# MOj0/vpt

Hardware: AMD Instinct MI355X
Metric: volume samples/s, MCM 512^3 @ 1920x1080 (higher is better)
Workload: dtype f32

## Files before the change

### vpt_amd/csrc/vpt_device.h

```cpp
#pragma once
#include <hip/hip_runtime.h>
#include <stdint.h>
#include "vpt_variants.h"

#define VPT_DEV __device__ __forceinline__

struct f3 { float x, y, z; };
struct f2 { float x, y; };

VPT_DEV float vmin(float a, float b) { return fminf(a, b); }
VPT_DEV float vmax(float a, float b) { return fmaxf(a, b); }
VPT_DEV float vclamp01(float x) { return vmin(vmax(x, 0.0f), 1.0f); }
VPT_DEV float mixf(float a, float b, float t) { return fmaf(b, t, a * (1.0f - t)); }
VPT_DEV f3 mix3(f3 a, f3 b, float t) { return f3{ mixf(a.x, b.x, t), mixf(a.y, b.y, t), mixf(a.z, b.z, t) }; }
VPT_DEV float dot3(f3 a, f3 b) { return fmaf(a.z, b.z, fmaf(a.y, b.y, a.x * b.x)); }
VPT_DEV float length3(f3 a) { return sqrtf(dot3(a, a)); }
VPT_DEV f3 sub3(f3 a, f3 b) { return f3{ a.x - b.x, a.y - b.y, a.z - b.z }; }
VPT_DEV f3 madd3(f3 p, float t, f3 d) { return f3{ fmaf(t, d.x, p.x), fmaf(t, d.y, p.y), fmaf(t, d.z, p.z) }; }
VPT_DEV float lerpf(float a, float b, float f) { return fmaf(f, b - a, a); }
VPT_DEV float4 lerp4(float4 a, float4 b, float f) {
    return make_float4(lerpf(a.x, b.x, f), lerpf(a.y, b.y, f), lerpf(a.z, b.z, f), lerpf(a.w, b.w, f));
}

VPT_DEV float rcp_nr(float x) {
// ... 347 lines not shown
        const uint32_t s0 = (uint32_t)(uintptr_t)a & 2u, s1 = ((uint32_t)(uintptr_t)a + 50u) & 2u;
        return norm16_blend<SNORM>(plane16_aligned(a - s0, s0), plane16_aligned(a + 50 - s1, s1), fx, fy, fz);
    }
    return norm16_blend<SNORM>(plane16(a), plane16(a + 50), fx, fy, fz);
}
template <bool WIDE>
VPT_DEV const uint8_t *record_addr(const DevVolume &v, const LdsTables &t, uint32_t x, uint32_t y, uint32_t z) {
    if (WIDE) return v.records + ((uint64_t)(t.tx[x] + t.ty[y]) * v.rec_col_bytes + (z << 2));
    return v.records + (uint32_t)(t.tx[x] + t.ty[y] + (z << 2));
}
VPT_DEV float record_blend(uint32_t lo, uint32_t hi, float fx, float fy, float fz) {
    float c000 = cvt_ubyte<0>(lo), c100 = cvt_ubyte<1>(lo), c010 = cvt_ubyte<2>(lo), c110 = cvt_ubyte<3>(lo);
    float c001 = cvt_ubyte<0>(hi), c101 = cvt_ubyte<1>(hi), c011 = cvt_ubyte<2>(hi), c111 = cvt_ubyte<3>(hi);
    float c00 = lerpf(c000, c100, fx), c10 = lerpf(c010, c110, fx);
    float c01 = lerpf(c001, c101, fx), c11 = lerpf(c011, c111, fx);
    float c0 = lerpf(c00, c10, fy), c1 = lerpf(c01, c11, fy);
    return lerpf(c0, c1, fz) * VPT_INV255;
}
VPT_DEV uint64_t record_load(const uint8_t *a) {
    uint64_t w;
    __builtin_memcpy(&w, __builtin_assume_aligned(a, 4), 8);
    return w;
}
VPT_DEV uint32_t boundary_cell(const DevVolume &v, f3 p, float &out_fa, float &out_fb) {
    const float fnx = v.fnx, fny = v.fny, fnz = v.fnz, hx = v.hx, hy = v.hy, hz = v.hz;
    const uint32_t face = v.atlas_face, sh = v.atlas_shift;
    const bool ox = (p.x > 1.0f) || (p.x < 0.0f);
    const bool oy = (p.y > 1.0f) || (p.y < 0.0f);
    const unsigned long long act = __builtin_amdgcn_ballot_w64(true);
    const unsigned long long bx = __builtin_amdgcn_ballot_w64(p.x > 1.0f) | __builtin_amdgcn_ballot_w64(p.x < 0.0f);
    const unsigned long long by = __builtin_amdgcn_ballot_w64(p.y > 1.0f) | __builtin_amdgcn_ballot_w64(p.y < 0.0f);
    uint32_t a, b, idx; float fa, fb;
    if (bx == act) {
        linear_cell(p.y, fny, hy, a, fa); linear_cell(p.z, fnz, hz, b, fb);
        idx = (p.x > 1.0f ? face : 0u) + ((b << sh) + a);
    } else if (bx == 0ull && by == act) {
        linear_cell(p.x, fnx, hx, a, fa); linear_cell(p.z, fnz, hz, b, fb);
        idx = (p.y > 1.0f ? 3u * face : 2u * face) + ((b << sh) + a);
    } else if (bx == 0ull && by == 0ull) {
        linear_cell(p.x, fnx, hx, a, fa); linear_cell(p.y, fny, hy, b, fb);
        idx = (p.z > 1.0f ? 5u * face : 4u * face) + ((b << sh) + a);
    } else {
        const bool oxy = ox || oy;
        const float pa = ox ? p.y : p.x, pb = oxy ? p.z : p.y;
        linear_cell(pa, ox ? fny : fnx, ox ? hy : hx, a, fa);
        linear_cell(pb, oxy ? fnz : fny, oxy ? hz : hy, b, fb);
        const float pk = ox ? p.x : (oy ? p.y : p.z);
        const uint32_t f = (ox ? 0u : (oy ? 2u : 4u)) + (pk > 1.0f ? 1u : 0u);
        idx = f * face + ((b << sh) + a);
    }
    out_fa = fa; out_fb = fb;
    return idx;
}
template <bool NEAREST>
VPT_DEV uint32_t boundary_cell_lane(const DevVolume &v, f3 p, float &out_fa, float &out_fb) {
    const float fnx = v.fnx, fny = v.fny, fnz = v.fnz, hx = v.hx, hy = v.hy, hz = v.hz;
    const bool ox = (p.x > 1.0f) || (p.x < 0.0f);
    const bool oy = (p.y > 1.0f) || (p.y < 0.0f);
    const bool oxy = ox || oy;
    const float pa = ox ? p.y : p.x, pb = oxy ? p.z : p.y;
    const float fna = ox ? fny : fnx, ha = ox ? hy : hx, fnb = oxy ? fnz : fny, hb = oxy ? hz : hy;
    uint32_t a, b; float fa = 0.0f, fb = 0.0f;
    if (NEAREST) { a = nearest_cell(pa, fna, ha); b = nearest_cell(pb, fnb, hb); }
    else { linear_cell(pa, fna, ha, a, fa); linear_cell(pb, fnb, hb, b, fb); }
    const float pk = ox ? p.x : (oy ? p.y : p.z);
    const uint32_t f = (ox ? 0u : (oy ? 2u : 4u)) + (pk > 1.0f ? 1u : 0u);
    out_fa = fa; out_fb = fb;
    return f * v.atlas_face + ((b << v.atlas_shift) + a);
}
template <bool SNORM = false>
VPT_DEV float boundary_blend(uint32_t w, float fa, float fb) {
    float c00 = byte_tap<SNORM, 0>(w), c10 = byte_tap<SNORM, 1>(w), c01 = byte_tap<SNORM, 2>(w), c11 = byte_tap<SNORM, 3>(w);
    const float r = lerpf(lerpf(c00, c10, fa), lerpf(c01, c11, fa), fb);
    return SNORM ? r : r * VPT_INV255;
}
template <int V>
VPT_DEV f2 sample_boundary_rg(const DevVolume &v, f3 p) {
    constexpr bool NEAREST = (V & VPT_V_NEAREST) != 0, RG = (V & VPT_V_RG) != 0, F32 = (V & (VPT_V_F32 | VPT_V_NORM16)) != 0, SNORM = (V & VPT_V_SNORM) != 0;
    float fa, fb;
    const uint32_t idx = boundary_cell_lane<NEAREST>(v, p, fa, fb);
    fa = cell_weight<V>(fa); fb = cell_weight<V>(fb);
    float val[2] = { 0.0f, 0.0f };
#pragma unroll
    for (int c = 0; c < (RG ? 2 : 1); c++) {
        const uint32_t cell = idx + (uint32_t)c * 6u * v.atlas_face;
        if (F32) {
            const float4 t = ((const float4 *)v.atlas)[cell];
            val[c] = NEAREST ? t.x : lerpf(lerpf(t.x, t.y, fa), lerpf(t.z, t.w, fa), fb);
        } else {
            const uint32_t w = v.atlas[cell];
            if (SNORM) val[c] = NEAREST ? snorm_byte<0>(w) : boundary_blend<true>(w, fa, fb);
            else val[c] = NEAREST ? cvt_ubyte<0>(w) * VPT_INV255 : boundary_blend(w, fa, fb);
        }
    }
    return f2{ val[0], val[1] };
}
VPT_DEV float sample_volume_boundary(const DevVolume &v, f3 p) {
    float fa, fb;
    const uint32_t idx = boundary_cell(v, p, fa, fb);
    return boundary_blend(v.atlas[idx], fa, fb);
}
template <int V>
VPT_DEV f2 sample_volume_rg(const DevVolume &v, const LdsTables &t, f3 p) {
    constexpr bool WIDE = (V & VPT_V_WIDE) != 0;
    constexpr bool RG = (V & VPT_V_RG) != 0;
    constexpr bool SNORM = (V & VPT_V_SNORM) != 0;
    if (V & VPT_V_NORM16) {
        if (V & VPT_V_NEAREST) {
            uint32_t x = nearest_cell(p.x, v.fnx, v.hx), y = nearest_cell(p.y, v.fny, v.hy), z = nearest_cell(p.z, v.fnz, v.hz);
            const uint16_t *b = (const uint16_t *)cell_addr<WIDE>(v, t, x, y, z);
            return f2{ norm16_word<SNORM, 0>(b[0]), RG ? norm16_word<SNORM, 0>(b[128]) : 0.0f };
        }
        uint32_t x, y, z; float fx, fy, fz;
        filter_cell<V>(p.x, v.fnx, v.hx, x, fx);
        filter_cell<V>(p.y, v.fny, v.hy, y, fy);
        filter_cell<V>(p.z, v.fnz, v.hz, z, fz);
        if ((V & VPT_V_ALIGNED) && !WIDE) {
            const uint32_t off = t.tx[x] + t.ty[y] + t.tz[z];
            return f2{ norm16_aligned_taps<SNORM>(v.bricks, off, fx, fy, fz), RG ? norm16_aligned_taps<SNORM>(v.bricks, off + 256u, fx, fy, fz) : 0.0f };
        }
        const uint8_t *a = cell_addr<WIDE>(v, t, x, y, z);
        return f2{ norm16_taps<V>(a, fx, fy, fz), RG ? norm16_taps<V>(a + 256, fx, fy, fz) : 0.0f };
    }
// ... 94 lines not shown
```

### vpt_amd/csrc/vpt_kernels_layout.h

```cpp
#pragma once
#include "vpt_kernels.h"


__global__ void __launch_bounds__(VPT_BLOCK) k_detile(PixMap pm, const uint8_t *src, uint8_t *dst, int elem) {
    Pix p = map_pixel(pm);
    if (!(p.i < pm.W && p.l < pm.local_h)) return;
    const uint8_t *s = src + (size_t)p.k * elem;
    uint8_t *d = dst + ((size_t)p.l * pm.W + p.i) * elem;
    for (int b = 0; b < elem; b++) d[b] = s[b];
}

__global__ void __launch_bounds__(VPT_BLOCK) k_detile_mcm3(PixMap pm, const f3 *src, float4 *dst) {
    Pix p = map_pixel(pm);
    if (!(p.i < pm.W && p.l < pm.local_h)) return;
    f3 v = src[p.k];
    dst[(size_t)p.l * pm.W + p.i] = make_float4(v.x, v.y, v.z, 0.0f);
}

__global__ void k_blit_block(uint8_t *vol, int nx, int ny, const uint8_t *blk, int x0, int y0, int z0, int bw, int bh, int bd, int ch) {
    size_t n = (size_t)bw * bh * bd;
    for (size_t t = (size_t)blockIdx.x * blockDim.x + threadIdx.x; t < n; t += (size_t)gridDim.x * blockDim.x) {
        int x = (int)(t % bw); size_t r = t / bw; int y = (int)(r % bh); int z = (int)(r / bh);
        size_t dst = (((size_t)(z0 + z) * ny + (y0 + y)) * nx + (x0 + x)) * ch;
        for (int c = 0; c < ch; c++) vol[dst + c] = blk[t * ch + c];
// ... 276 lines not shown
        case 6: { uint32_t st = __float_as_uint(in[t]); r = random_uniform(st); } break;
        case 7: r = __uint_as_float((uint32_t)to_half_bits(in[t])); break;
        case 8: r = rcp_nr(in[t]); break;
        case 9: r = rsqrt_nr(in[t]); break;
        case 10: r = vmin(in[2 * t], in[2 * t + 1]); break;
        case 11: r = vmax(in[2 * t], in[2 * t + 1]); break;
        case 12: r = vpt_logf_uniform(in[t]); break;
        case 13: r = rcp_nrz(in[t]); break;
        case 14: r = sqrt_nr(in[t]); break;
        case 15: r = vpt_expf(in[t]); break;
        case 16: r = vpt_powf(in[2 * t], in[2 * t + 1]); break;
    }
    out[t] = r;
}
template <int V>
__global__ void __launch_bounds__(VPT_BLOCK) k_probe_sample_boundary(PassArgs a, const float *xyz, float4 *out, size_t n) {
    extern __shared__ float4 lds_raw[];
    LdsTables t = stage_lds<(V & VPT_V_WIDE) != 0>(lds_raw, a);
    size_t i = (size_t)blockIdx.x * blockDim.x + threadIdx.x;
    if (i >= n) return;
    const f3 q = { xyz[3 * i], xyz[3 * i + 1], xyz[3 * i + 2] };
    const bool oob = (vmax(vmax(q.x, q.y), q.z) > 1.0f) || (vmin(vmin(q.x, q.y), q.z) < 0.0f);
    if (!oob) { out[i] = sample_volume_color<V>(a, t, q); return; }
    const f2 rg = sample_boundary_rg<V>(a.vol, q);
    out[i] = (V & VPT_V_RG) ? sample_tf2d(a.tf, a.tf_w, a.tf_h, rg.x, rg.y) : sample_tf(t.tf, a.tf_fw, a.tf_hi, rg.x);
}
template <int V>
__global__ void __launch_bounds__(VPT_BLOCK) k_probe_sample(PassArgs a, const float *xyz, float4 *out, size_t n) {
    extern __shared__ float4 lds_raw[];
    LdsTables t = stage_lds<(V & VPT_V_WIDE) != 0>(lds_raw, a);
    size_t i = (size_t)blockIdx.x * blockDim.x + threadIdx.x;
    if (i >= n) return;
    out[i] = sample_volume_color<V>(a, t, f3{ xyz[3 * i], xyz[3 * i + 1], xyz[3 * i + 2] });
}
```

### vpt_amd/csrc/vpt_kernels_mcm.h

```cpp
#pragma once
#include "vpt_kernels.h"

struct Photon {
    f3 position, direction, transmittance, radiance;
    uint32_t bounces, samples;
};
template <bool NOBLUR = false>
VPT_DEV void unproject_rand(uint32_t &state, float px, float py, const PassArgs &a, f3 from0, f3 &from, f3 &to) {
    if (NOBLUR || a.blur == 0.0f) {
        random_uniform(state); random_uniform(state);
        from = from0;
    } else {
        f2 d = random_disk(state);
        from = dehomogenize(mat4_mul_point(a.mvp_inv, px + d.x * a.blur, py + d.y * a.blur, -1.0f));
    }
    float sx = random_uniform(state), sy = random_uniform(state);
    float ax = fmaf(sx, 2.0f, -1.0f) * a.inv_w;
    float ay = fmaf(sy, 2.0f, -1.0f) * a.inv_h;
    to = dehomogenize(mat4_mul_point(a.mvp_inv, px + ax, py + ay, 1.0f));
}
VPT_DEV f3 unproject_near(float px, float py, const PassArgs &a) {
    return dehomogenize(mat4_mul_point(a.mvp_inv, px + 0.0f, py + 0.0f, -1.0f));
}
VPT_DEV f3 photon_start(f3 from, f3 dir) {
// ... 34 lines not shown

#ifdef VPT_MCM_PLAIN_KERNELS
__global__ void __launch_bounds__(VPT_BLOCK) k_mcm_reset(PassArgs a) {
    Pix p = map_pixel(a.pm);
    if (!p.tile) return;
    Photon ph;
    if (p.valid) {
        float px = ndc_col(a.pm, p.i), py = ndc_row(a.pm, p.j);
        uint32_t state = hash3(__float_as_uint(px), __float_as_uint(py), __float_as_uint(a.seed));
        reset_photon(state, ph, px, py, a, unproject_near(px, py, a));
    } else {
        ph.position = f3{ 0.0f, 0.0f, 0.0f };
        ph.direction = f3{ 0.0f, 0.0f, 1.0f };
    }
    ((f3 *)a.st0)[p.k] = ph.position;
    a.st1[p.k] = make_float4(ph.direction.x, ph.direction.y, ph.direction.z, 0.0f);
    ((f3 *)a.st2)[p.k] = f3{ 1.0f, 1.0f, 1.0f };
    a.st3[p.k] = make_float4(1.0f, 1.0f, 1.0f, 0.0f);
}
#endif

#ifdef VPT_EVENT_TIMING
#define VPT_TIMING_WAVES 16384
struct EventClock { unsigned long long prev, start; unsigned long long acc[8]; };
VPT_DEV void ev_start(EventClock &c) { for (int i = 0; i < 8; i++) c.acc[i] = 0ull; c.prev = wall_clock64(); c.start = c.prev; }
#define EV_MARK(c, slot, WAIT) do { asm volatile(WAIT ::: "memory"); const unsigned long long n_ = wall_clock64(); (c).acc[slot] += n_ - (c).prev; (c).prev = n_; } while (0)
#define EV_PIN3(v) asm volatile("" : "+v"((v).x), "+v"((v).y), "+v"((v).z))
VPT_DEV void ev_flush(const EventClock &c, unsigned long long *out) {
    if (((int)threadIdx.x & 63) == 0 && out) {
        unsigned long long *slot = out + (((size_t)blockIdx.x * 4 + (threadIdx.x >> 6)) & (VPT_TIMING_WAVES - 1)) * 16;
        for (int i = 0; i < 8; i++) slot[i] += c.acc[i];
        slot[8] += 1ull;
        slot[9] = c.start; slot[10] = c.prev;
    }
}
#define EV_PARAM , EventClock &evc
#define EV_ARG , evc
#define EV_LOCAL EventClock evc; ev_start(evc);
#else
#define EV_MARK(c, slot, WAIT) do { } while (0)
#define EV_PIN3(v) do { } while (0)
#define EV_PARAM
#define EV_ARG
#define EV_LOCAL
#endif
struct SampleLoads { uint32_t aw; uint64_t w0, w1; float f0, f1, f2; uint32_t atlas; };
template <int V>
VPT_DEV SampleLoads mcm_sample_issue(const PassArgs &a, const LdsTables &t, f3 p, bool oob) {
    constexpr bool WIDE = (V & VPT_V_WIDE) != 0;
    SampleLoads s;
    s.aw = 0u; s.w0 = 0ull; s.w1 = 0ull; s.f0 = 0.0f; s.f1 = 0.0f; s.f2 = 0.0f;
    asm volatile("" : "+v"(s.w0), "+v"(s.w1), "+v"(s.aw));
    const bool at = oob && a.vol.atlas != nullptr;
    if (at) {
        s.aw = a.vol.atlas[boundary_cell(a.vol, p, s.f0, s.f1)];
    } else {
        uint32_t x, y, z;
        linear_cell(p.x, a.vol.fnx, a.vol.hx, x, s.f0);
        linear_cell(p.y, a.vol.fny, a.vol.hy, y, s.f1);
        linear_cell(p.z, a.vol.fnz, a.vol.hz, z, s.f2);
        if (V & VPT_V_REC) {
            s.w0 = record_load(record_addr<WIDE>(a.vol, t, x, y, z));
        } else {
            const uint8_t *b = cell_addr<WIDE>(a.vol, t, x, y, z);
            __builtin_memcpy(&s.w0, b, 8);
            __builtin_memcpy(&s.w1, b + 25, 8);
        }
    }
    s.atlas = at ? 1u : 0u;
    asm volatile("" : "+v"(s.atlas));
    return s;
}
template <int V>
VPT_DEV float4 mcm_sample_finish(const PassArgs &a, const LdsTables &t, const SampleLoads &s) {
    float r;
    if (!s.atlas) {
        if (V & VPT_V_REC) r = record_blend((uint32_t)s.w0, (uint32_t)(s.w0 >> 32), s.f0, s.f1, s.f2);
        else r = trilinear_blend((uint32_t)s.w0, (uint32_t)(s.w0 >> 32), (uint32_t)s.w1, (uint32_t)(s.w1 >> 32), s.f0, s.f1, s.f2);
// ... 318 lines not shown
    photon_store(a, p.k, ph);
    if (FUSE_RENDER) store_frame(a, p, pack_half4(ph.radiance.x, ph.radiance.y, ph.radiance.z, 1.0f));
#ifdef VPT_EVENT_TIMING
    EV_MARK(evc, 6, "s_waitcnt vmcnt(0)");
    ev_flush(evc, a.violations);
#endif
}
template <bool FUSE_RENDER, int V>
__global__ void __launch_bounds__(VPT_BLOCK) __attribute__((amdgpu_waves_per_eu(5, 8))) k_mcm_integrate_early(PassArgs a) {
    frame_select(a, 0);
    Pix p = map_pixel(a.pm);
    PhotonState st;
    if (p.tile) st = photon_load(a, p.k);
    extern __shared__ float4 lds_raw[];
    LdsTables t = stage_lds<(V & VPT_V_WIDE) != 0, (V & VPT_V_REC) != 0>(lds_raw, a);
    if (!p.valid) return;
    float px = ndc_col(a.pm, p.i), py = ndc_row(a.pm, p.j);
    Photon ph = photon_unpack(st);
    if (V & VPT_V_FAST) mcm_events_fast_early<V & ~VPT_V_FAST>(a, t, ph, px, py);
    else mcm_events_early<V>(a, t, ph, px, py);
    photon_store(a, p.k, ph);
    if (FUSE_RENDER) store_frame(a, p, pack_half4(ph.radiance.x, ph.radiance.y, ph.radiance.z, 1.0f));
}
VPT_DEV const float4 *stage_tf(float4 *lds, const PassArgs &a) {
    const int nthreads = (int)blockDim.x;
    for (int t = (int)threadIdx.x; t < a.tf_w; t += nthreads) {
        float4 v = a.tf[t], n = a.tf[min(t + 1, a.tf_w - 1)];
        lds[2 * t] = v;
        lds[2 * t + 1] = make_float4(n.x - v.x, n.y - v.y, n.z - v.z, n.w - v.w);
    }
    __syncthreads();
    return lds;
}
struct MissLoad { uint32_t aw; float fa, fb; };
template <bool CHECK>
VPT_DEV MissLoad miss_sample_issue(const PassArgs &a, f3 q, unsigned long long *violations) {
    MissLoad l;
    l.aw = a.vol.atlas[boundary_cell(a.vol, q, l.fa, l.fb)];
    if (CHECK) {
        const bool oob = (vmax(vmax(q.x, q.y), q.z) > 1.0f) || (vmin(vmin(q.x, q.y), q.z) < 0.0f);
        if (!oob) atomicAdd(violations, 1ull);
    }
    return l;
}
VPT_DEV void miss_sample_finish(const PassArgs &a, const float4 *tf, const MissLoad &l) {
    float4 vs = sample_tf(tf, a.tf_fw, a.tf_hi, boundary_blend(l.aw, l.fa, l.fb));
    asm volatile("" : "+v"(vs.w));
}
template <int V>
VPT_DEV void miss_sample_any(const PassArgs &a, const float4 *tf, f3 q) {
    const f2 rg = sample_boundary_rg<V>(a.vol, q);
    float4 vs = (V & VPT_V_RG) ? sample_tf2d(a.tf, a.tf_w, a.tf_h, rg.x, rg.y) : sample_tf(tf, a.tf_fw, a.tf_hi, rg.x);
    asm volatile("" : "+v"(vs.w));
    if (a.miss_verify) {
        const bool oob = (vmax(vmax(q.x, q.y), q.z) > 1.0f) || (vmin(vmin(q.x, q.y), q.z) < 0.0f);
        if (!oob) atomicAdd(a.violations, 1ull);
    }
}
template <int V, bool CHECK, bool LATE, bool DEPOSIT = true>
VPT_DEV void mcm_events_miss(const PassArgs &a, const float4 *tf, Photon &ph, float px, float py, f3 from0) {
    uint32_t state = hash3(__float_as_uint(ndc_to_uv(px)), __float_as_uint(ndc_to_uv(py)), __float_as_uint(a.seed));
    for (uint32_t s = 0u; s < a.steps; s++) {
        float dist = random_exponential(state, a.inv_extinction);
        ph.position = madd3(ph.position, dist, ph.direction);
        constexpr bool OTHER = (V & (VPT_V_NEAREST | VPT_V_RG | VPT_V_F32 | VPT_V_SNORM)) != 0;
        MissLoad l = { 0u, 0.0f, 0.0f };
        if (OTHER) miss_sample_any<V>(a, tf, ph.position);
        else l = miss_sample_issue<CHECK>(a, ph.position, a.violations);
        if (!LATE && !OTHER) miss_sample_finish(a, tf, l);
        random_uniform(state);
        if (DEPOSIT) {
            float4 env = sample_environment(a.env, ph.direction);
            photon_deposit(ph, f3{ env.x, env.y, env.z });
        }
        reset_photon<true>(state, ph, px, py, a, from0);
        if (LATE && !OTHER) miss_sample_finish(a, tf, l);
    }
}
template <int V, bool CHECK, bool LATE, bool DEPOSIT = true>
VPT_DEV void mcm_events_miss_fast(const PassArgs &a, const float4 *tf, const FastPixel &c, Photon &ph, float px, float py) {
    const float ld = -0.6931471805599453f * a.inv_extinction, ld32 = -32.0f * ld;
    uint32_t state = hash3(__float_as_uint(ndc_to_uv(px)), __float_as_uint(ndc_to_uv(py)), __float_as_uint(a.seed));
    for (uint32_t s = 0u; s < a.steps; s++) {
        float dist = fmaf(hw_log2(pcg_float(state)), ld, ld32);
        ph.position = madd3(ph.position, dist, ph.direction);
        constexpr bool OTHER = (V & (VPT_V_NEAREST | VPT_V_RG | VPT_V_F32 | VPT_V_SNORM)) != 0;
        MissLoad l = { 0u, 0.0f, 0.0f };
        if (OTHER) miss_sample_any<V>(a, tf, ph.position);
        else l = miss_sample_issue<CHECK>(a, ph.position, a.violations);
        if (!LATE && !OTHER) miss_sample_finish(a, tf, l);
        state = pcg(state);
        f3 rad = { 0.0f, 0.0f, 0.0f };
        if (DEPOSIT) { float4 env = sample_environment(a.env, ph.direction); rad = f3{ env.x, env.y, env.z }; }
        fast_path_end<true, DEPOSIT>(a, c, state, ph, rad, px, py);
        if (LATE && !OTHER) miss_sample_finish(a, tf, l);
    }
}
template <bool FUSE_RENDER, int V, bool CHECK, bool LATE>
__global__ void __launch_bounds__(VPT_BLOCK)
__attribute__((amdgpu_waves_per_eu(((V & (VPT_V_NEAREST | VPT_V_RG | VPT_V_F32 | VPT_V_SNORM)) && !(V & VPT_V_FAST)) ? 7 : 8, 8))) k_mcm_miss(PassArgs a) {
    frame_select(a, 0);
    Pix p = map_pixel(a.pm);
    float4 s1 = make_float4(0.0f, 0.0f, 1.0f, 0.0f), s3 = make_float4(0.0f, 0.0f, 0.0f, 0.0f);
    f3 s0 = { 0.0f, 0.0f, 0.0f };
    if (p.tile) {
        s1 = a.st1[p.k]; s3 = a.st3[p.k];
        if (a.miss_load_pos) s0 = ((const f3 *)a.st0)[p.k];
    }
    extern __shared__ float4 lds_raw[];
    const float4 *tf = stage_tf(lds_raw, a);
    if (!p.valid) return;
    const float px = ndc_col(a.pm, p.i), py = ndc_row(a.pm, p.j);
    Photon ph;
    ph.direction = f3{ s1.x, s1.y, s1.z };
    ph.bounces = 0u;
    ph.transmittance = f3{ 1.0f, 1.0f, 1.0f };
    ph.radiance = f3{ s3.x, s3.y, s3.z };
    ph.samples = (uint32_t)(s3.w + 0.5f);
    if (V & VPT_V_FAST) {
        const FastPixel c = fast_pixel(a, px, py);
        ph.position = a.miss_load_pos ? s0 : photon_start_fast(c.from0, ph.direction);
        mcm_events_miss_fast<V & ~VPT_V_FAST, CHECK, LATE>(a, tf, c, ph, px, py);
    } else {
        const f3 from0 = unproject_near(px, py, a);
        ph.position = a.miss_load_pos ? s0 : photon_start(from0, ph.direction);
        mcm_events_miss<V, CHECK, LATE>(a, tf, ph, px, py, from0);
    }
    a.st1[p.k] = make_float4(ph.direction.x, ph.direction.y, ph.direction.z, 0.0f);
    a.st3[p.k] = make_float4(ph.radiance.x, ph.radiance.y, ph.radiance.z, (float)ph.samples);
    if (FUSE_RENDER) store_frame(a, p, pack_half4(ph.radiance.x, ph.radiance.y, ph.radiance.z, 1.0f));
}
template <int V, bool CHECK, bool LATE>
__global__ void __launch_bounds__(VPT_BLOCK) __attribute__((amdgpu_waves_per_eu(8, 8))) k_mcm_miss_settled(PassArgs a) {
    frame_select(a, 0);
    Pix p = map_pixel(a.pm);
    float4 s1 = make_float4(0.0f, 0.0f, 1.0f, 0.0f);
    f3 s0 = { 0.0f, 0.0f, 0.0f };
    if (p.tile) {
        s1 = a.st1[p.k];
        if (a.miss_load_pos) s0 = ((const f3 *)a.st0)[p.k];
    }
    extern __shared__ float4 lds_raw[];
    const float4 *tf = stage_tf(lds_raw, a);
    if (!p.valid) return;
    const float px = ndc_col(a.pm, p.i), py = ndc_row(a.pm, p.j);
    Photon ph;
    ph.direction = f3{ s1.x, s1.y, s1.z };
    ph.bounces = 0u;
    ph.transmittance = f3{ 1.0f, 1.0f, 1.0f };
    ph.radiance = f3{ 0.0f, 0.0f, 0.0f };
    ph.samples = 0u;
    if (V & VPT_V_FAST) {
        const FastPixel c = fast_pixel(a, px, py);
        ph.position = a.miss_load_pos ? s0 : photon_start_fast(c.from0, ph.direction);
        mcm_events_miss_fast<V & ~VPT_V_FAST, CHECK, LATE, false>(a, tf, c, ph, px, py);
    } else {
        const f3 from0 = unproject_near(px, py, a);
        ph.position = a.miss_load_pos ? s0 : photon_start(from0, ph.direction);
        mcm_events_miss<V, CHECK, LATE, false>(a, tf, ph, px, py, from0);
    }
    a.st1[p.k] = make_float4(ph.direction.x, ph.direction.y, ph.direction.z, 0.0f);
}
template <bool FAST>
__global__ void __launch_bounds__(VPT_BLOCK) k_mcm_materialize(PassArgs a, uint32_t pending) {
    Pix p = map_pixel(a.pm);
    if (!p.valid) return;
    if (pending) a.st3[p.k].w = (float)((uint32_t)(a.st3[p.k].w + 0.5f) + pending);
    const float px = ndc_col(a.pm, p.i), py = ndc_row(a.pm, p.j);
    const float4 s1 = a.st1[p.k];
    const f3 dir = { s1.x, s1.y, s1.z };
    f3 pos;
    if (FAST) pos = photon_start_fast(fast_pixel(a, px, py).from0, dir);
    else pos = photon_start(unproject_near(px, py, a), dir);
    ((f3 *)a.st0)[p.k] = pos;
    ((f3 *)a.st2)[p.k] = f3{ 1.0f, 1.0f, 1.0f };
}

template <int V, bool FRAMES>
VPT_DEV void mcm_multi_body(PassArgs &a, uint32_t npasses, uint2 *ring, uint32_t slot_pixels) {
    extern __shared__ float4 lds_raw[];
    LdsTables t = stage_lds<(V & VPT_V_WIDE) != 0, (V & VPT_V_REC) != 0>(lds_raw, a);
    Pix p = map_pixel(a.pm);
    if (!p.valid) return;
    float px = ndc_col(a.pm, p.i), py = ndc_row(a.pm, p.j);
// ... 56 lines not shown
    Pix p = map_pixel(a.pm);
    float4 s1 = make_float4(0.0f, 0.0f, 1.0f, 0.0f), s3 = make_float4(0.0f, 0.0f, 0.0f, 0.0f);
    f3 s0 = { 0.0f, 0.0f, 0.0f };
    if (p.tile) {
        s1 = a.st1[p.k]; s3 = a.st3[p.k];
        if (a.miss_load_pos) s0 = ((const f3 *)a.st0)[p.k];
    }
    extern __shared__ float4 lds_raw[];
    const float4 *tf = stage_tf(lds_raw, a);
    if (!p.valid) return;
    const float px = ndc_col(a.pm, p.i), py = ndc_row(a.pm, p.j);
    Photon ph;
    ph.direction = f3{ s1.x, s1.y, s1.z };
    ph.bounces = 0u;
    ph.transmittance = f3{ 1.0f, 1.0f, 1.0f };
    ph.radiance = f3{ s3.x, s3.y, s3.z };
    ph.samples = (uint32_t)(s3.w + 0.5f);
    size_t texel = (size_t)p.l * a.pm.W + p.i;
    if (V & VPT_V_FAST) {
        const FastPixel c = fast_pixel(a, px, py);
        ph.position = a.miss_load_pos ? s0 : photon_start_fast(c.from0, ph.direction);
        for (uint32_t f = 0; f < nframes; f++) {
            a.seed = fs.seed[f];
            mcm_events_miss_fast<V & ~VPT_V_FAST, false, LATE>(a, tf, c, ph, px, py);
            bucket_store<DISPLAY>(a, ring, texel, pack_half4(ph.radiance.x, ph.radiance.y, ph.radiance.z, 1.0f));
            texel += slot_pixels;
        }
    } else {
        const f3 from0 = unproject_near(px, py, a);
        ph.position = a.miss_load_pos ? s0 : photon_start(from0, ph.direction);
        for (uint32_t f = 0; f < nframes; f++) {
            a.seed = fs.seed[f];
            mcm_events_miss<V, false, LATE>(a, tf, ph, px, py, from0);
            bucket_store<DISPLAY>(a, ring, texel, pack_half4(ph.radiance.x, ph.radiance.y, ph.radiance.z, 1.0f));
            texel += slot_pixels;
        }
    }
    a.st1[p.k] = make_float4(ph.direction.x, ph.direction.y, ph.direction.z, 0.0f);
    a.st3[p.k] = make_float4(ph.radiance.x, ph.radiance.y, ph.radiance.z, (float)ph.samples);
    if (a.render) store_frame_texel(&a.render[(size_t)p.l * a.pm.W + p.i], pack_half4(ph.radiance.x, ph.radiance.y, ph.radiance.z, 1.0f));
}
#ifdef VPT_MCM_PLAIN_KERNELS
__global__ void __launch_bounds__(VPT_BLOCK) k_mcm_render(PassArgs a) {
    Pix p = map_pixel(a.pm);
    if (!p.valid) return;
    float4 r = a.st3[p.k];
    a.render[(size_t)p.l * a.pm.W + p.i] = pack_half4(r.x, r.y, r.z, 1.0f);
}
#endif
```

### vpt_amd/csrc/vpt_mcm.hip

```cpp
#include "vpt_mcm_select.h"
#define VPT_MCM_PLAIN_KERNELS
#include "vpt_kernels_mcm.h"

#ifdef VPT_EVENT_TIMING
#define VPT_TIMING_ARG(part, hit) do { if (hit) (part).violations = timing; } while (0)
#else
#define VPT_TIMING_ARG(part, hit) do { } while (0)
#endif
#ifdef VPT_EVENT_TIMING
static unsigned long long *g_timing = nullptr;
static unsigned long long *timing_buffer(vpt_renderer *r) {
    if (!g_timing) {
        if (hipMalloc(&g_timing, (size_t)VPT_TIMING_WAVES * 16 * sizeof(unsigned long long)) != hipSuccess) { g_timing = nullptr; return nullptr; }
        hipMemsetAsync(g_timing, 0, (size_t)VPT_TIMING_WAVES * 16 * sizeof(unsigned long long), r->ctx->stream);
    }
    return g_timing;
}
#endif
static bool mcm_classes_usable(const vpt_renderer *r, const PassArgs &a) {
    return r->cls.enabled && r->cls.valid && a.blur == 0.0f && memcmp(r->cls.mvp, a.mvp_inv.m, sizeof(r->cls.mvp)) == 0;
}
static bool mcm_classes_runnable(const vpt_renderer *r, const PassArgs &a) {
    return a.vol.atlas != nullptr && !r->mcm_persistent && !(r->vol->snorm && !r->vol->norm16);
}
static bool mcm_plain_volume(const vpt_renderer *r) { return (variant_of(r) & ~VPT_V_WIDE) == 0 && unsigned_r8(r->vol); }
template <bool FUSE> static PassKernel format_miss_kernel(int v, bool fast) {
    return dispatch_variant<VPT_V_NEAREST | VPT_V_RG | VPT_V_F32>(
        v, [&](auto F) { return fast ? (PassKernel)k_mcm_miss<FUSE, F() | VPT_V_FAST, false, true> : (PassKernel)k_mcm_miss<FUSE, F(), false, true>; }, no_pass_kernel);
}
int mcm_materialize(vpt_renderer *r) {
    if (!r->cls.stale) return VPT_OK;
    VPT_TRY(join_side(r));
    HIP_TRY(hipSetDevice(r->ctx->device));
    PassArgs a;
    VPT_TRY(make_args(r, nullptr, false, &a));
    memcpy(a.mvp_inv.m, r->cls.mvp, sizeof(r->cls.mvp));
    a.pm.tile_list = r->cls.list + r->cls.n_hit; a.pm.list_n = r->cls.n_miss;
    if (r->cls.n_miss > 0) {
        if (r->cls.stale_fast) hipLaunchKernelGGL(k_mcm_materialize<true>, dim3((unsigned)r->cls.n_miss), dim3(VPT_BLOCK), 0, r->ctx->stream, a, r->cls.pending);
// ... 92 lines not shown
    TileClasses &c = r->cls;
    const bool wanted = c.settled_opt && !(vm & ~VPT_V_WIDE) && c.n_miss > 0 && !c.env_changed && !r->no_split && settle_env_usable(r) &&
                        a.steps >= 1u && c.events >= 1 && c.events + a.steps < (1ull << 24);
    if (wanted && c.settle == 0 && c.pending == 0) VPT_TRY(settle_probe(r));
    const bool settled = wanted && c.settle == 1 && (!FUSE || (a.tm_table == nullptr && settled_destination(r, a.render)));
    if (settled) {
        if (check) km = fast ? (late ? (PassKernel)k_mcm_miss_settled<VPT_V_FAST, true, true> : (PassKernel)k_mcm_miss_settled<VPT_V_FAST, true, false>)
                             : (PassKernel)k_mcm_miss_settled<0, true, true>;
        else km = fast ? (late ? (PassKernel)k_mcm_miss_settled<VPT_V_FAST, false, true> : (PassKernel)k_mcm_miss_settled<VPT_V_FAST, false, false>)
                       : (PassKernel)k_mcm_miss_settled<0, false, true>;
    } else {
        VPT_TRY(mcm_catch_up(r));
        if (FUSE && c.n_miss > 0 && a.steps >= 1u && c.settle != 2) {
            if (c.settle == 0) { c.n_complete = 0; c.complete_events = c.events + a.steps; }
            if (!settled_destination(r, a.render) && c.n_complete < VPT_COMPLETE_DESTS) c.complete[c.n_complete++] = (const void *)a.render;
        }
    }
    const size_t lds_hit = lds_bytes(r), lds_miss = (size_t)r->tf_w * 2 * sizeof(float4);
    VPT_TRY(lds_prepare((const void *)kh, lds_hit));
    const int k = split_allowed(r) ? r->split : 1;
    struct Part { PassKernel kernel; const uint32_t *list; int n; size_t lds; };
    Part parts[VPT_MAX_SPLIT]; int np = 0;
#ifdef VPT_EVENT_TIMING
    unsigned long long *const timing = timing_buffer(r);
#endif
    const int hit_parts = r->cls.n_hit > 0 ? 1 : 0;
    const int miss_parts = std::max(1, k - hit_parts);
    for (int i = 0; i < hit_parts; i++) {
        const int h0 = (int)((long long)r->cls.n_hit * i / hit_parts), h1 = (int)((long long)r->cls.n_hit * (i + 1) / hit_parts);
        if (h1 > h0) parts[np++] = Part{ kh, r->cls.list + h0, h1 - h0, lds_hit };
    }
    for (int i = 0; i < miss_parts; i++) {
        const int m0 = (int)((long long)r->cls.n_miss * i / miss_parts), m1 = (int)((long long)r->cls.n_miss * (i + 1) / miss_parts);
        if (m1 > m0) parts[np++] = Part{ km, r->cls.list + r->cls.n_hit + m0, m1 - m0, lds_miss };
    }
    VPT_TRY(streams_deal(r, Deal{ DEAL_LISTS, k == 1 ? 1 : std::max(np, 1) }));
    auto part_args = [&](int i) {
        PassArgs part = a;
        part.pm.tile_list = parts[i].list; part.pm.list_n = parts[i].n; part.miss_load_pos = r->cls.stale ? 0u : 1u; part.violations = r->cls.violations;
        part.miss_verify = check ? 1u : 0u;
        VPT_TIMING_ARG(part, i < hit_parts);
        return part;
    };
    if (k == 1) {
        for (int i = 0; i < np; i++) {
            const PassArgs part = part_args(i);
            const hipEvent_t e1 = i >= hit_parts && i == np - 1 ? side_events_begin(r, r->ctx->stream) : nullptr;
// ... 120 lines not shown
int mcm_reset(vpt_renderer *r, const PassArgs &a, const vpt_uniforms *u) {
    LAUNCH(k_mcm_reset, r, a, 0);
    HIP_TRY(hipGetLastError());
    return mcm_classify(r, u);
}
int mcm_pass(vpt_renderer *r, const PassArgs &a, bool fuse_render) {
    return fuse_render ? launch_mcm_pass<true>(r, a) : launch_mcm_pass<false>(r, a);
}
int mcm_render_frame(vpt_renderer *r, const PassArgs &a) {
    if (r->streams.busy() && r->streams.last == Deal{ DEAL_LISTS, 2 } && r->cls.valid && r->cls.n_hit > 0 && r->cls.n_miss > 0 &&
        !r->target_is_callers && !r->stop_events) {
        PassArgs part = a;
        part.pm.tile_list = r->cls.list; part.pm.list_n = r->cls.n_hit;
        hipLaunchKernelGGL(k_mcm_render, dim3((unsigned)r->cls.n_hit), dim3(VPT_BLOCK), 0, r->ctx->stream, part);
        part.pm.tile_list = r->cls.list + r->cls.n_hit; part.pm.list_n = r->cls.n_miss;
        hipLaunchKernelGGL(k_mcm_render, dim3((unsigned)r->cls.n_miss), dim3(VPT_BLOCK), 0, range_stream(r, 1), part);
        return VPT_OK;
    }
    VPT_TRY(join_side(r));
    LAUNCH(k_mcm_render, r, a, 0);
    return VPT_OK;
}
#ifdef VPT_EVENT_TIMING
extern "C" VPT_API int vpt_probe_event_timing(vpt_renderer *r, uint64_t *out9) {
    if (!r || !out9 || !g_timing) return fail(VPT_ERR_INVALID, "no timing buffer (run a classified pass first)");
    VPT_TRY(join_side(r));
    HIP_TRY(hipSetDevice(r->ctx->device));
    std::vector<unsigned long long> host((size_t)VPT_TIMING_WAVES * 16);
    HIP_TRY(hipMemcpyAsync(host.data(), g_timing, host.size() * 8, hipMemcpyDeviceToHost, r->ctx->stream));
    HIP_TRY(hipMemsetAsync(g_timing, 0, host.size() * 8, r->ctx->stream));
    HIP_TRY(hipStreamSynchronize(r->ctx->stream));
    for (int k = 0; k < 9; k++) out9[k] = 0;
    for (size_t w = 0; w < VPT_TIMING_WAVES; w++) for (int k = 0; k < 9; k++) out9[k] += host[w * 16 + k];
    std::vector<unsigned long long> st, en;
    unsigned long long t0 = ~0ull;
    for (size_t w = 0; w < VPT_TIMING_WAVES; w++) if (host[w * 16 + 8]) { st.push_back(host[w * 16 + 9]); en.push_back(host[w * 16 + 10]); t0 = std::min(t0, host[w * 16 + 9]); }
    for (int k = 9; k < 17; k++) out9[k] = 0;
    if (!st.empty()) {
        std::sort(st.begin(), st.end()); std::sort(en.begin(), en.end());
        const size_t n = st.size();
        out9[9] = n; out9[10] = st[n / 2] - t0; out9[11] = st[n * 9 / 10] - t0; out9[12] = st[n - 1] - t0;
        out9[13] = en[n / 10] - t0; out9[14] = en[n / 2] - t0; out9[15] = en[n * 9 / 10] - t0; out9[16] = en[n - 1] - t0;
    }
    return VPT_OK;
}
#endif
```

Before: 221.8 billion.

## Restructure miss kernel prologue, add per-axis boundary ballots, and miss timing probes

Adds a templated boundary_cell that checks each axis with a wave-wide ballot, taking uniform fast paths when the whole wave is out of bounds on a single axis. Atlas reads now go through an aligned memcpy helper. The miss kernels now do per-pixel setup (including the RNG seed) before the LDS barrier, so that work overlaps the transfer-function staging, and out-of-range lanes return only after the barrier. It also adds an event-timing buffer and probe for miss kernels, and a plain-format shortcut in the sample kernel. The extra ballot for the z axis adds a little work on divergent waves.

```diff
diff --git a/vpt_amd/csrc/vpt_device.h b/vpt_amd/csrc/vpt_device.h
--- a/vpt_amd/csrc/vpt_device.h
+++ b/vpt_amd/csrc/vpt_device.h
@@ -393,11 +393,10 @@
     __builtin_memcpy(&w, __builtin_assume_aligned(a, 4), 8);
     return w;
 }
+template <bool ANY_AXIS = true>
 VPT_DEV uint32_t boundary_cell(const DevVolume &v, f3 p, float &out_fa, float &out_fb) {
     const float fnx = v.fnx, fny = v.fny, fnz = v.fnz, hx = v.hx, hy = v.hy, hz = v.hz;
     const uint32_t face = v.atlas_face, sh = v.atlas_shift;
-    const bool ox = (p.x > 1.0f) || (p.x < 0.0f);
-    const bool oy = (p.y > 1.0f) || (p.y < 0.0f);
     const unsigned long long act = __builtin_amdgcn_ballot_w64(true);
     const unsigned long long bx = __builtin_amdgcn_ballot_w64(p.x > 1.0f) | __builtin_amdgcn_ballot_w64(p.x < 0.0f);
     const unsigned long long by = __builtin_amdgcn_ballot_w64(p.y > 1.0f) | __builtin_amdgcn_ballot_w64(p.y < 0.0f);
@@ -405,13 +404,15 @@
     if (bx == act) {
         linear_cell(p.y, fny, hy, a, fa); linear_cell(p.z, fnz, hz, b, fb);
         idx = (p.x > 1.0f ? face : 0u) + ((b << sh) + a);
-    } else if (bx == 0ull && by == act) {
+    } else if ((ANY_AXIS || bx == 0ull) && by == act) {
         linear_cell(p.x, fnx, hx, a, fa); linear_cell(p.z, fnz, hz, b, fb);
         idx = (p.y > 1.0f ? 3u * face : 2u * face) + ((b << sh) + a);
-    } else if (bx == 0ull && by == 0ull) {
+    } else if (ANY_AXIS ? (__builtin_amdgcn_ballot_w64(p.z > 1.0f) | __builtin_amdgcn_ballot_w64(p.z < 0.0f)) == act : (bx == 0ull && by == 0ull)) {
         linear_cell(p.x, fnx, hx, a, fa); linear_cell(p.y, fny, hy, b, fb);
         idx = (p.z > 1.0f ? 5u * face : 4u * face) + ((b << sh) + a);
     } else {
+        const bool ox = (p.x > 1.0f) || (p.x < 0.0f);
+        const bool oy = (p.y > 1.0f) || (p.y < 0.0f);
         const bool oxy = ox || oy;
         const float pa = ox ? p.y : p.x, pb = oxy ? p.z : p.y;
         linear_cell(pa, ox ? fny : fnx, ox ? hy : hx, a, fa);
@@ -438,6 +439,11 @@
     const uint32_t f = (ox ? 0u : (oy ? 2u : 4u)) + (pk > 1.0f ? 1u : 0u);
     out_fa = fa; out_fb = fb;
     return f * v.atlas_face + ((b << v.atlas_shift) + a);
+}
+VPT_DEV uint32_t atlas_dword(const uint32_t *atlas, uint32_t idx) {
+    uint32_t w;
+    __builtin_memcpy(&w, __builtin_assume_aligned((const uint8_t *)atlas + (idx << 2), 4), 4);
+    return w;
 }
 template <bool SNORM = false>
 VPT_DEV float boundary_blend(uint32_t w, float fa, float fb) {
@@ -469,7 +475,7 @@
 VPT_DEV float sample_volume_boundary(const DevVolume &v, f3 p) {
     float fa, fb;
     const uint32_t idx = boundary_cell(v, p, fa, fb);
-    return boundary_blend(v.atlas[idx], fa, fb);
+    return boundary_blend(atlas_dword(v.atlas, idx), fa, fb);
 }
 template <int V>
 VPT_DEV f2 sample_volume_rg(const DevVolume &v, const LdsTables &t, f3 p) {
diff --git a/vpt_amd/csrc/vpt_kernels_layout.h b/vpt_amd/csrc/vpt_kernels_layout.h
--- a/vpt_amd/csrc/vpt_kernels_layout.h
+++ b/vpt_amd/csrc/vpt_kernels_layout.h
@@ -322,7 +322,8 @@
     const f3 q = { xyz[3 * i], xyz[3 * i + 1], xyz[3 * i + 2] };
     const bool oob = (vmax(vmax(q.x, q.y), q.z) > 1.0f) || (vmin(vmin(q.x, q.y), q.z) < 0.0f);
     if (!oob) { out[i] = sample_volume_color<V>(a, t, q); return; }
-    const f2 rg = sample_boundary_rg<V>(a.vol, q);
+    constexpr bool PLAIN = !(V & (VPT_V_NEAREST | VPT_V_RG | VPT_V_F32 | VPT_V_SNORM | VPT_V_QCUBIC | VPT_V_NORM16));
+    const f2 rg = PLAIN ? f2{ sample_volume_boundary(a.vol, q), 0.0f } : sample_boundary_rg<V>(a.vol, q);
     out[i] = (V & VPT_V_RG) ? sample_tf2d(a.tf, a.tf_w, a.tf_h, rg.x, rg.y) : sample_tf(t.tf, a.tf_fw, a.tf_hi, rg.x);
 }
 template <int V>
diff --git a/vpt_amd/csrc/vpt_kernels_mcm.h b/vpt_amd/csrc/vpt_kernels_mcm.h
--- a/vpt_amd/csrc/vpt_kernels_mcm.h
+++ b/vpt_amd/csrc/vpt_kernels_mcm.h
@@ -80,13 +80,14 @@
 
 #ifdef VPT_EVENT_TIMING
 #define VPT_TIMING_WAVES 16384
+#define VPT_TIMING_MISS_WAVES 32768
 struct EventClock { unsigned long long prev, start; unsigned long long acc[8]; };
 VPT_DEV void ev_start(EventClock &c) { for (int i = 0; i < 8; i++) c.acc[i] = 0ull; c.prev = wall_clock64(); c.start = c.prev; }
 #define EV_MARK(c, slot, WAIT) do { asm volatile(WAIT ::: "memory"); const unsigned long long n_ = wall_clock64(); (c).acc[slot] += n_ - (c).prev; (c).prev = n_; } while (0)
 #define EV_PIN3(v) asm volatile("" : "+v"((v).x), "+v"((v).y), "+v"((v).z))
-VPT_DEV void ev_flush(const EventClock &c, unsigned long long *out) {
+VPT_DEV void ev_flush(const EventClock &c, unsigned long long *out, size_t waves = VPT_TIMING_WAVES) {
     if (((int)threadIdx.x & 63) == 0 && out) {
-        unsigned long long *slot = out + (((size_t)blockIdx.x * 4 + (threadIdx.x >> 6)) & (VPT_TIMING_WAVES - 1)) * 16;
+        unsigned long long *slot = out + (((size_t)blockIdx.x * 4 + (threadIdx.x >> 6)) & (waves - 1)) * 16;
         for (int i = 0; i < 8; i++) slot[i] += c.acc[i];
         slot[8] += 1ull;
         slot[9] = c.start; slot[10] = c.prev;
@@ -111,7 +112,7 @@
     asm volatile("" : "+v"(s.w0), "+v"(s.w1), "+v"(s.aw));
     const bool at = oob && a.vol.atlas != nullptr;
     if (at) {
-        s.aw = a.vol.atlas[boundary_cell(a.vol, p, s.f0, s.f1)];
+        s.aw = atlas_dword(a.vol.atlas, boundary_cell<false>(a.vol, p, s.f0, s.f1));
     } else {
         uint32_t x, y, z;
         linear_cell(p.x, a.vol.fnx, a.vol.hx, x, s.f0);
@@ -476,13 +477,17 @@
     photon_store(a, p.k, ph);
     if (FUSE_RENDER) store_frame(a, p, pack_half4(ph.radiance.x, ph.radiance.y, ph.radiance.z, 1.0f));
 }
-VPT_DEV const float4 *stage_tf(float4 *lds, const PassArgs &a) {
+VPT_DEV const float4 *stage_tf_fill(float4 *lds, const PassArgs &a) {
     const int nthreads = (int)blockDim.x;
     for (int t = (int)threadIdx.x; t < a.tf_w; t += nthreads) {
         float4 v = a.tf[t], n = a.tf[min(t + 1, a.tf_w - 1)];
         lds[2 * t] = v;
         lds[2 * t + 1] = make_float4(n.x - v.x, n.y - v.y, n.z - v.z, n.w - v.w);
     }
+    return lds;
+}
+VPT_DEV const float4 *stage_tf(float4 *lds, const PassArgs &a) {
+    stage_tf_fill(lds, a);
     __syncthreads();
     return lds;
 }
@@ -490,7 +495,7 @@
 template <bool CHECK>
 VPT_DEV MissLoad miss_sample_issue(const PassArgs &a, f3 q, unsigned long long *violations) {
     MissLoad l;
-    l.aw = a.vol.atlas[boundary_cell(a.vol, q, l.fa, l.fb)];
+    l.aw = atlas_dword(a.vol.atlas, boundary_cell(a.vol, q, l.fa, l.fb));
     if (CHECK) {
         const bool oob = (vmax(vmax(q.x, q.y), q.z) > 1.0f) || (vmin(vmin(q.x, q.y), q.z) < 0.0f);
         if (!oob) atomicAdd(violations, 1ull);
@@ -511,9 +516,11 @@
         if (!oob) atomicAdd(a.violations, 1ull);
     }
 }
+VPT_DEV uint32_t pass_seed(float px, float py, float seed) {
+    return hash3(__float_as_uint(ndc_to_uv(px)), __float_as_uint(ndc_to_uv(py)), __float_as_uint(seed));
+}
 template <int V, bool CHECK, bool LATE, bool DEPOSIT = true>
-VPT_DEV void mcm_events_miss(const PassArgs &a, const float4 *tf, Photon &ph, float px, float py, f3 from0) {
-    uint32_t state = hash3(__float_as_uint(ndc_to_uv(px)), __float_as_uint(ndc_to_uv(py)), __float_as_uint(a.seed));
+VPT_DEV void mcm_events_miss(const PassArgs &a, const float4 *tf, Photon &ph, float px, float py, f3 from0, uint32_t state) {
     for (uint32_t s = 0u; s < a.steps; s++) {
         float dist = random_exponential(state, a.inv_extinction);
         ph.position = madd3(ph.position, dist, ph.direction);
@@ -532,9 +539,8 @@
     }
 }
 template <int V, bool CHECK, bool LATE, bool DEPOSIT = true>
-VPT_DEV void mcm_events_miss_fast(const PassArgs &a, const float4 *tf, const FastPixel &c, Photon &ph, float px, float py) {
+VPT_DEV void mcm_events_miss_fast(const PassArgs &a, const float4 *tf, const FastPixel &c, Photon &ph, float px, float py, uint32_t state) {
     const float ld = -0.6931471805599453f * a.inv_extinction, ld32 = -32.0f * ld;
-    uint32_t state = hash3(__float_as_uint(ndc_to_uv(px)), __float_as_uint(ndc_to_uv(py)), __float_as_uint(a.seed));
     for (uint32_t s = 0u; s < a.steps; s++) {
         float dist = fmaf(hw_log2(pcg_float(state)), ld, ld32);
         ph.position = madd3(ph.position, dist, ph.direction);
@@ -550,70 +556,104 @@
         if (LATE && !OTHER) miss_sample_finish(a, tf, l);
     }
 }
+struct MissPixel { FastPixel c; f3 from0; uint32_t state; };
+template <bool FAST>
+VPT_DEV MissPixel miss_pixel_start(const PassArgs &a, float px, float py, float4 s1, f3 s0, Photon &ph) {
+    MissPixel m;
+    ph.direction = f3{ s1.x, s1.y, s1.z };
+    ph.bounces = 0u;
+    ph.transmittance = f3{ 1.0f, 1.0f, 1.0f };
+    if (FAST) {
+        m.c = fast_pixel(a, px, py);
+        m.from0 = m.c.from0;
+        ph.position = a.miss_load_pos ? s0 : photon_start_fast(m.c.from0, ph.direction);
+    } else {
+        m.from0 = unproject_near(px, py, a);
+        ph.position = a.miss_load_pos ? s0 : photon_start(m.from0, ph.direction);
+    }
+    m.state = pass_seed(px, py, a.seed);
+    asm volatile("" : "+v"(ph.position.x), "+v"(ph.position.y), "+v"(ph.position.z), "+v"(m.state));
+    return m;
+}
+#ifdef VPT_EVENT_TIMING
+#define EV_MISS_MARK(evc, slot, WAIT) EV_MARK(evc, slot, WAIT)
+#define EV_MISS_PIN(x) asm volatile("" : "+v"(x))
+#define EV_MISS_BEGIN(evc, ph) do { EV_PIN3((ph).position); EV_MARK(evc, 5, "s_waitcnt vmcnt(0) lgkmcnt(0)"); } while (0)
+#define EV_MISS_EVENTS(evc, ph) do { EV_PIN3((ph).direction); EV_MARK(evc, 0, "s_waitcnt vmcnt(0) lgkmcnt(0)"); } while (0)
+#define EV_MISS_END(evc, a) do { EV_MARK(evc, 6, "s_waitcnt vmcnt(0)"); ev_flush(evc, CHECK ? nullptr : (a).violations, VPT_TIMING_MISS_WAVES); } while (0)
+#else
+#define EV_MISS_MARK(evc, slot, WAIT) do { } while (0)
+#define EV_MISS_PIN(x) do { } while (0)
+#define EV_MISS_BEGIN(evc, ph) do { } while (0)
+#define EV_MISS_EVENTS(evc, ph) do { } while (0)
+#define EV_MISS_END(evc, a) do { } while (0)
+#endif
 template <bool FUSE_RENDER, int V, bool CHECK, bool LATE>
 __global__ void __launch_bounds__(VPT_BLOCK)
 __attribute__((amdgpu_waves_per_eu(((V & (VPT_V_NEAREST | VPT_V_RG | VPT_V_F32 | VPT_V_SNORM)) && !(V & VPT_V_FAST)) ? 7 : 8, 8))) k_mcm_miss(PassArgs a) {
+    EV_LOCAL
     frame_select(a, 0);
     Pix p = map_pixel(a.pm);
+    EV_MISS_PIN(p.k); EV_MISS_MARK(evc, 1, "s_waitcnt lgkmcnt(0)");
     float4 s1 = make_float4(0.0f, 0.0f, 1.0f, 0.0f), s3 = make_float4(0.0f, 0.0f, 0.0f, 0.0f);
     f3 s0 = { 0.0f, 0.0f, 0.0f };
+    float px = 0.0f, py = 0.0f;
     if (p.tile) {
         s1 = a.st1[p.k]; s3 = a.st3[p.k];
         if (a.miss_load_pos) s0 = ((const f3 *)a.st0)[p.k];
     }
+    if (p.valid) { px = ndc_col(a.pm, p.i); py = ndc_row(a.pm, p.j); }
     extern __shared__ float4 lds_raw[];
-    const float4 *tf = stage_tf(lds_raw, a);
-    if (!p.valid) return;
-    const float px = ndc_col(a.pm, p.i), py = ndc_row(a.pm, p.j);
+    const float4 *tf = stage_tf_fill(lds_raw, a);
+    EV_MISS_MARK(evc, 2, "s_waitcnt vmcnt(0)");
     Photon ph;
-    ph.direction = f3{ s1.x, s1.y, s1.z };
-    ph.bounces = 0u;
-    ph.transmittance = f3{ 1.0f, 1.0f, 1.0f };
+    const MissPixel m = miss_pixel_start<(V & VPT_V_FAST) != 0>(a, px, py, s1, s0, ph);
+    EV_MISS_MARK(evc, 3, "");
+    __syncthreads();
+    EV_MISS_MARK(evc, 4, "");
+    if (!p.valid) return;
     ph.radiance = f3{ s3.x, s3.y, s3.z };
     ph.samples = (uint32_t)(s3.w + 0.5f);
-    if (V & VPT_V_FAST) {
-        const FastPixel c = fast_pixel(a, px, py);
-        ph.position = a.miss_load_pos ? s0 : photon_start_fast(c.from0, ph.direction);
-        mcm_events_miss_fast<V & ~VPT_V_FAST, CHECK, LATE>(a, tf, c, ph, px, py);
-    } else {
-        const f3 from0 = unproject_near(px, py, a);
-        ph.position = a.miss_load_pos ? s0 : photon_start(from0, ph.direction);
-        mcm_events_miss<V, CHECK, LATE>(a, tf, ph, px, py, from0);
-    }
+    EV_MISS_BEGIN(evc, ph);
+    if (V & VPT_V_FAST) mcm_events_miss_fast<V & ~VPT_V_FAST, CHECK, LATE>(a, tf, m.c, ph, px, py, m.state);
+    else mcm_events_miss<V, CHECK, LATE>(a, tf, ph, px, py, m.from0, m.state);
+    EV_MISS_EVENTS(evc, ph);
     a.st1[p.k] = make_float4(ph.direction.x, ph.direction.y, ph.direction.z, 0.0f);
     a.st3[p.k] = make_float4(ph.radiance.x, ph.radiance.y, ph.radiance.z, (float)ph.samples);
     if (FUSE_RENDER) store_frame(a, p, pack_half4(ph.radiance.x, ph.radiance.y, ph.radiance.z, 1.0f));
+    EV_MISS_END(evc, a);
 }
 template <int V, bool CHECK, bool LATE>
 __global__ void __launch_bounds__(VPT_BLOCK) __attribute__((amdgpu_waves_per_eu(8, 8))) k_mcm_miss_settled(PassArgs a) {
+    EV_LOCAL
     frame_select(a, 0);
     Pix p = map_pixel(a.pm);
+    EV_MISS_PIN(p.k); EV_MISS_MARK(evc, 1, "s_waitcnt lgkmcnt(0)");
     float4 s1 = make_float4(0.0f, 0.0f, 1.0f, 0.0f);
     f3 s0 = { 0.0f, 0.0f, 0.0f };
+    float px = 0.0f, py = 0.0f;
     if (p.tile) {
         s1 = a.st1[p.k];
         if (a.miss_load_pos) s0 = ((const f3 *)a.st0)[p.k];
     }
+    if (p.valid) { px = ndc_col(a.pm, p.i); py = ndc_row(a.pm, p.j); }
     extern __shared__ float4 lds_raw[];
-    const float4 *tf = stage_tf(lds_raw, a);
-    if (!p.valid) return;
-    const float px = ndc_col(a.pm, p.i), py = ndc_row(a.pm, p.j);
+    const float4 *tf = stage_tf_fill(lds_raw, a);
+    EV_MISS_MARK(evc, 2, "s_waitcnt vmcnt(0)");
     Photon ph;
-    ph.direction = f3{ s1.x, s1.y, s1.z };
-    ph.bounces = 0u;
-    ph.transmittance = f3{ 1.0f, 1.0f, 1.0f };
+    const MissPixel m = miss_pixel_start<(V & VPT_V_FAST) != 0>(a, px, py, s1, s0, ph);
+    EV_MISS_MARK(evc, 3, "");
+    __syncthreads();
+    EV_MISS_MARK(evc, 4, "");
+    if (!p.valid) return;
     ph.radiance = f3{ 0.0f, 0.0f, 0.0f };
     ph.samples = 0u;
-    if (V & VPT_V_FAST) {
-        const FastPixel c = fast_pixel(a, px, py);
-        ph.position = a.miss_load_pos ? s0 : photon_start_fast(c.from0, ph.direction);
-        mcm_events_miss_fast<V & ~VPT_V_FAST, CHECK, LATE, false>(a, tf, c, ph, px, py);
-    } else {
-        const f3 from0 = unproject_near(px, py, a);
-        ph.position = a.miss_load_pos ? s0 : photon_start(from0, ph.direction);
-        mcm_events_miss<V, CHECK, LATE, false>(a, tf, ph, px, py, from0);
-    }
+    EV_MISS_BEGIN(evc, ph);
+    if (V & VPT_V_FAST) mcm_events_miss_fast<V & ~VPT_V_FAST, CHECK, LATE, false>(a, tf, m.c, ph, px, py, m.state);
+    else mcm_events_miss<V, CHECK, LATE, false>(a, tf, ph, px, py, m.from0, m.state);
+    EV_MISS_EVENTS(evc, ph);
     a.st1[p.k] = make_float4(ph.direction.x, ph.direction.y, ph.direction.z, 0.0f);
+    EV_MISS_END(evc, a);
 }
 template <bool FAST>
 __global__ void __launch_bounds__(VPT_BLOCK) k_mcm_materialize(PassArgs a, uint32_t pending) {
@@ -716,7 +756,7 @@
         ph.position = a.miss_load_pos ? s0 : photon_start_fast(c.from0, ph.direction);
         for (uint32_t f = 0; f < nframes; f++) {
             a.seed = fs.seed[f];
-            mcm_events_miss_fast<V & ~VPT_V_FAST, false, LATE>(a, tf, c, ph, px, py);
+            mcm_events_miss_fast<V & ~VPT_V_FAST, false, LATE>(a, tf, c, ph, px, py, pass_seed(px, py, a.seed));
             bucket_store<DISPLAY>(a, ring, texel, pack_half4(ph.radiance.x, ph.radiance.y, ph.radiance.z, 1.0f));
             texel += slot_pixels;
         }
@@ -725,7 +765,7 @@
         ph.position = a.miss_load_pos ? s0 : photon_start(from0, ph.direction);
         for (uint32_t f = 0; f < nframes; f++) {
             a.seed = fs.seed[f];
-            mcm_events_miss<V, false, LATE>(a, tf, ph, px, py, from0);
+            mcm_events_miss<V, false, LATE>(a, tf, ph, px, py, from0, pass_seed(px, py, a.seed));
             bucket_store<DISPLAY>(a, ring, texel, pack_half4(ph.radiance.x, ph.radiance.y, ph.radiance.z, 1.0f));
             texel += slot_pixels;
         }
diff --git a/vpt_amd/csrc/vpt_mcm.hip b/vpt_amd/csrc/vpt_mcm.hip
--- a/vpt_amd/csrc/vpt_mcm.hip
+++ b/vpt_amd/csrc/vpt_mcm.hip
@@ -3,18 +3,21 @@
 #include "vpt_kernels_mcm.h"
 
 #ifdef VPT_EVENT_TIMING
-#define VPT_TIMING_ARG(part, hit) do { if (hit) (part).violations = timing; } while (0)
+#define VPT_TIMING_ARG(part, hit) do { if (hit) (part).violations = timing; else if (!check) (part).violations = timing_miss; } while (0)
 #else
 #define VPT_TIMING_ARG(part, hit) do { } while (0)
 #endif
 #ifdef VPT_EVENT_TIMING
-static unsigned long long *g_timing = nullptr;
-static unsigned long long *timing_buffer(vpt_renderer *r) {
-    if (!g_timing) {
-        if (hipMalloc(&g_timing, (size_t)VPT_TIMING_WAVES * 16 * sizeof(unsigned long long)) != hipSuccess) { g_timing = nullptr; return nullptr; }
-        hipMemsetAsync(g_timing, 0, (size_t)VPT_TIMING_WAVES * 16 * sizeof(unsigned long long), r->ctx->stream);
-    }
-    return g_timing;
+static unsigned long long *g_timing[2] = { nullptr, nullptr };
+static const size_t g_timing_waves[2] = { VPT_TIMING_WAVES, VPT_TIMING_MISS_WAVES };
+static unsigned long long *timing_buffer(vpt_renderer *r, int which) {
+    if (!g_timing[which]) {
+        const size_t bytes = g_timing_waves[which] * 16 * sizeof(unsigned long long);
+        if (hipMalloc(&g_timing[which], bytes) != hipSuccess) { g_timing[which] = nullptr; return nullptr; }
+        hipMemsetAsync(g_timing[which], 0, bytes, r->ctx->stream);
+        hipStreamSynchronize(r->ctx->stream);
+    }
+    return g_timing[which];
 }
 #endif
 static bool mcm_classes_usable(const vpt_renderer *r, const PassArgs &a) {
@@ -153,7 +156,7 @@
     struct Part { PassKernel kernel; const uint32_t *list; int n; size_t lds; };
     Part parts[VPT_MAX_SPLIT]; int np = 0;
 #ifdef VPT_EVENT_TIMING
-    unsigned long long *const timing = timing_buffer(r);
+    unsigned long long *const timing = timing_buffer(r, 0), *const timing_miss = timing_buffer(r, 1);
 #endif
     const int hit_parts = r->cls.n_hit > 0 ? 1 : 0;
     const int miss_parts = std::max(1, k - hit_parts);
@@ -320,19 +323,20 @@
     return VPT_OK;
 }
 #ifdef VPT_EVENT_TIMING
-extern "C" VPT_API int vpt_probe_event_timing(vpt_renderer *r, uint64_t *out9) {
-    if (!r || !out9 || !g_timing) return fail(VPT_ERR_INVALID, "no timing buffer (run a classified pass first)");
+static int probe_timing(vpt_renderer *r, int which, uint64_t *out9) {
+    if (!r || !out9 || !g_timing[which]) return fail(VPT_ERR_INVALID, "no timing buffer (run a classified pass first)");
     VPT_TRY(join_side(r));
     HIP_TRY(hipSetDevice(r->ctx->device));
-    std::vector<unsigned long long> host((size_t)VPT_TIMING_WAVES * 16);
-    HIP_TRY(hipMemcpyAsync(host.data(), g_timing, host.size() * 8, hipMemcpyDeviceToHost, r->ctx->stream));
-    HIP_TRY(hipMemsetAsync(g_timing, 0, host.size() * 8, r->ctx->stream));
+    const size_t waves = g_timing_waves[which];
+    std::vector<unsigned long long> host(waves * 16);
+    HIP_TRY(hipMemcpyAsync(host.data(), g_timing[which], host.size() * 8, hipMemcpyDeviceToHost, r->ctx->stream));
+    HIP_TRY(hipMemsetAsync(g_timing[which], 0, host.size() * 8, r->ctx->stream));
     HIP_TRY(hipStreamSynchronize(r->ctx->stream));
     for (int k = 0; k < 9; k++) out9[k] = 0;
-    for (size_t w = 0; w < VPT_TIMING_WAVES; w++) for (int k = 0; k < 9; k++) out9[k] += host[w * 16 + k];
+    for (size_t w = 0; w < waves; w++) for (int k = 0; k < 9; k++) out9[k] += host[w * 16 + k];
     std::vector<unsigned long long> st, en;
     unsigned long long t0 = ~0ull;
-    for (size_t w = 0; w < VPT_TIMING_WAVES; w++) if (host[w * 16 + 8]) { st.push_back(host[w * 16 + 9]); en.push_back(host[w * 16 + 10]); t0 = std::min(t0, host[w * 16 + 9]); }
+    for (size_t w = 0; w < waves; w++) if (host[w * 16 + 8]) { st.push_back(host[w * 16 + 9]); en.push_back(host[w * 16 + 10]); t0 = std::min(t0, host[w * 16 + 9]); }
     for (int k = 9; k < 17; k++) out9[k] = 0;
     if (!st.empty()) {
         std::sort(st.begin(), st.end()); std::sort(en.begin(), en.end());
@@ -342,4 +346,6 @@
     }
     return VPT_OK;
 }
+extern "C" VPT_API int vpt_probe_event_timing(vpt_renderer *r, uint64_t *out9) { return probe_timing(r, 0, out9); }
+extern "C" VPT_API int vpt_probe_miss_timing(vpt_renderer *r, uint64_t *out9) { return probe_timing(r, 1, out9); }
 #endif
```

Result: faster. 229.0 billion, median of 6 (+3.3%).
